# thomasgilgenast/hic3defdr

Hardware: AMD Instinct MI355X
Metric: pixels/sec through estimate_disp+lrt, 4 reps @10kb; max-|Δq| vs reference (higher is better)
Workload: dtype f64; 1 GPU; cfg2: per GPU 1 chrom x 20000 bins, 4 reps (2+2), dist_thresh_max 250, estimate_disp (qcml) + lrt on HBM-resident inputs; disp_pixels_rank0=3757837, disp_pixels_total=3757837, parallelism=dp1 (chromosome shards; in-kernel Brent searches)

## Files before the change

### hic3defdr_amd/csrc/h3d_api.hip

```cpp
#include <hip/hip_runtime.h>
#include <hipcub/hipcub.hpp>

#include <algorithm>
#include <chrono>
#include <cstdarg>
#include <cstdio>
#include <cstdlib>
#include <cstring>
#include <map>
#include <string>
#include <thread>
#include <type_traits>
#include <vector>

#include "h3d.h"
#include "h3d_ctx.h"
#include "h3d_errors.h"
#include "h3d_host.h"
#include "h3d_kernels.h"

using namespace h3d;
using namespace h3dint;
using h3derr::fail;

// ... 377 lines not shown
  int64_t n = 0;
  int R = 0, C = 0, D = 0;
  h3d_allreduce_fn reduce = nullptr;
  void* user = nullptr;
  const TableReq* treq = nullptr;
  int S = 0, mslot = 0;
  bool nll_full = false;
  std::vector<int> nrep;
  std::vector<int32_t> rep_idx;
  bool dev_tables = false;
  bool dual = false;
  HostStamps stamp;
  int32_t *raw_s = nullptr, *dist_s = nullptr;
  double *f_s = nullptr, *pd = nullptr;
  int64_t* d_seg = nullptr;
  std::vector<int64_t> seg_start;
  int n_chunks = 0;
  size_t max_items = 0;
  int64_t *d_cs = nullptr, *d_lpx = nullptr;
  int32_t *d_cl = nullptr, *d_cd = nullptr, *d_scb = nullptr, *d_sce = nullptr;
  int32_t *d_nrep = nullptr, *d_repidx = nullptr;
  SegState* d_st = nullptr;
  int32_t *d_list = nullptr, *d_meta = nullptr, *d_slb = nullptr, *d_sle = nullptr;
  double *d_partial = nullptr, *d_total = nullptr, *d_res = nullptr;
  int *d_flags = nullptr, *d_bad = nullptr, *d_queue = nullptr;
  GangTables gang;
  int32_t* h_meta = nullptr;
  double* h_resd = nullptr;
  SegState* h_sst = nullptr;
  int* h_bad = nullptr;
  bool have_res = false;
};

template <int M, bool NLL, bool kFull = false>
void launch_disp_work(const DispCall& c) {
  h3d_ctx* ctx = c.ctx;
  auto launch = [&](auto k) {
    hipLaunchKernelGGL(k, dim3(work_grid(ctx, k, c.max_items)), dim3(kBlock), 0, c.s, c.raw_s,
                       c.f_s, c.pd, c.n, c.d_cs, c.d_cl, c.d_cd, c.C, c.d_repidx, c.d_nrep,
                       c.d_st, c.d_flags, c.d_list, c.d_meta, c.d_partial, ctx->eq_static8);
  };
  {
    ProfScope ps(ctx, "disp_work", 0, 1);
    launch(k_disp_work<M, (M <= 8 ? 4 : 1), kEqualize, NLL, kFull>);
  }
  if constexpr (NLL) {
    ProfScope ps(ctx, "disp_nll", 0);
    launch(k_disp_work<M, 1, kNll>);
  }
}

template <typename K>
int radix_sort_pairs(h3d_ctx* ctx, const K* keys_in, K* keys_out, const int32_t* vals_in,
                     int32_t* vals_out, int64_t n, int begin_bit, int end_bit) {
  return cub_call(ctx, "cub_tmp", [&](void* tmp, size_t& bytes) {
    return hipcub::DeviceRadixSort::SortPairs(tmp, bytes, keys_in, keys_out, vals_in, vals_out,
                                              (int)n, begin_bit, end_bit, ctx->stream);
  });
}

int validate_and_plan(DispCall& c, const int32_t* cond_of_rep, int estimator) {
  h3d_ctx* ctx = c.ctx;
  const int64_t n = c.n;
  if (n < 0 || c.D < 1) return fail(H3D_EARG, "n=%lld D=%d", (long long)n, c.D);
  if (n > 0 && (!c.d_raw || !c.d_f || !c.d_dist)) return fail(H3D_EARG, "null device input");
  if (n >= (int64_t)1 << 31) return fail(H3D_EARG, "n=%lld exceeds 2^31 pixels per call", (long long)n);
  if (estimator != H3D_EST_QCML)
    return fail(H3D_EARG, "estimator %d: only qcml runs on the GPU path (the reference's cml/mme divide an int64 array in place and raise)", estimator);
  if (int rc = check_cond(cond_of_rep, c.R, c.C, &c.nrep, &c.rep_idx)) return rc;
  HIP_TRY(hipSetDevice(ctx->device));
  if (std::getenv("H3D_DEBUG")) {
    const hipError_t pe = hipGetLastError();
    if (pe != hipSuccess)
      fprintf(stderr, "[h3d] estimate_disp entry: pending HIP error %s\n", hipGetErrorString(pe));
  }
  c.s = ctx->stream;
  c.S = c.D * c.C;
// ... 290 lines not shown
int qcml_single_rank(DispCall& c) {
  h3d_ctx* ctx = c.ctx;
  if (c.n == 0) {
    Scratch sc{ctx};
    c.d_seg = sc.get<int64_t>("seg_start", c.D + 1);
    if (!sc.ok) return fail(H3D_ENOMEM, "brent scratch");
    HIP_TRY(hipMemsetAsync(c.d_seg, 0, (c.D + 1) * 8, c.s));
  }
  bool use_gang = ctx->brent_gang == 2 && c.n > 0;
  if (use_gang) {
    const int grc = with_width(c.mslot, false, [&](auto m, auto) {
      return gang_setup<decltype(m)::value>(ctx, c.seg_start, c.D, c.C, &c.gang);
    });
    if (grc == 1) use_gang = false;
    else if (grc) return grc;
  }
  int rounds = 0, batch = 5;
  while (true) {
    for (int b = 0; b < batch; ++b) {
      dbg_launch("before qcml iteration");
      with_width(c.mslot, c.nll_full, [&](auto m, auto full) {
        constexpr int M = decltype(m)::value;
        constexpr bool kFull = decltype(full)::value;
        auto brent = [&](const int32_t* gate_meta, int live_min, const int* gang_abort) {
          launch_brent<M, kFull>(ctx, c.pd, c.n, c.d_seg, c.S, c.C, c.d_repidx, c.d_nrep,
                                 c.d_st, c.d_flags, c.d_res, c.d_queue, gate_meta, live_min,
                                 gang_abort, true);
        };
        auto gang = [&](const int32_t* gate_meta, int live_max) {
          launch_brent_gang<M, kFull>(ctx, c.pd, c.n, c.d_seg, c.S, c.C, c.d_repidx, c.d_nrep,
                                      c.d_st, c.d_flags, c.d_res, c.d_queue + 1, c.gang,
                                      gate_meta, live_max, true);
        };
        launch_disp_work<M, false, kFull>(c);
        dbg_launch("equalize");
        if (c.dual) {
          brent(c.d_meta, ctx->n_cu, c.gang.abort);
          dbg_launch("k_brent (dual)");
          gang(c.d_meta, ctx->n_cu);
          dbg_launch("k_brent_gang (dual)");
        } else if (use_gang) {
          gang(nullptr, 0);
        } else {
          brent(nullptr, 0, nullptr);
        }
      });
      launch_seg_update(c, 0, 0);
      ++rounds;
    }
    const bool gangs = use_gang || c.dual;
    if (int rc = poll_single_rank(c, gangs)) return rc;
    if (std::getenv("H3D_DEBUG"))
      fprintf(stderr, "[h3d] qcml iterations=%d live_segments=%d gang=%d abort=%d\n", rounds,
              c.h_meta[3], use_gang ? 1 : c.dual ? 2 : 0, gangs ? c.h_meta[4] : 0);
    if (c.dual && c.h_meta[4]) {
      c.dual = false;
      ctx->gang_aborts += 1;
    }
    if (use_gang && c.h_meta[4]) {
      use_gang = false;
      ctx->gang_aborts += 1;
      continue;
    }
    if (c.h_meta[3] == 0) return 0;
    if (rounds > 2000) return fail(H3D_ENOCONV, "estimate_disp did not terminate");
    batch = 2;
  }
// ... 110 lines not shown
  }
  if (device < 0 || device >= n) {
    fail(H3D_EARG, "device %d of %d", device, n);
    return nullptr;
  }
  hipDeviceProp_t prop;
  if (hipGetDeviceProperties(&prop, device) != hipSuccess) {
    fail(H3D_EHIP, "hipGetDeviceProperties failed");
    return nullptr;
  }
  if (std::strncmp(prop.gcnArchName, "gfx950", 6) != 0) {
    fail(H3D_ENODEV, "device %d is %s, libh3d is built for gfx950", device,
         prop.gcnArchName);
    return nullptr;
  }
  if (hipSetDevice(device) != hipSuccess) {
    fail(H3D_EHIP, "hipSetDevice failed");
    return nullptr;
  }
  h3d_ctx* ctx = new h3d_ctx();
  ctx->device = device;
  ctx->n_cu = prop.multiProcessorCount;
  if (hipStreamCreateWithFlags(&ctx->own, hipStreamNonBlocking) != hipSuccess) {
    delete ctx;
    fail(H3D_EHIP, "stream create failed");
    return nullptr;
  }
  ctx->stream = ctx->own;
  if (const char* e = std::getenv("H3D_EQ_STATIC8"))
    ctx->eq_static8 = std::max(0, std::min(8, std::atoi(e)));
  if (const char* e = std::getenv("H3D_BRENT")) ctx->brent_gang = std::atoi(e);
  if (const char* e = std::getenv("H3D_BRENT_LDS_KB")) ctx->brent_lds_kb = std::atoi(e);
  if (const char* e = std::getenv("H3D_NLL_FULL")) ctx->nll_full = std::atoi(e);
  if (const char* e = std::getenv("H3D_GANG_P")) ctx->gang_px = std::atoi(e);
  if (hipMalloc((void**)&ctx->work_count, 2 * sizeof(unsigned long long)) != hipSuccess ||
      hipMemset(ctx->work_count, 0, 2 * sizeof(unsigned long long)) != hipSuccess) {
    (void)hipStreamDestroy(ctx->own);
    delete ctx;
    fail(H3D_ENOMEM, "counter allocation failed");
    return nullptr;
  }
  return ctx;
}

void h3d_close(h3d_ctx* ctx) {
  if (!ctx) return;
  (void)hipSetDevice(ctx->device);
  (void)hipStreamSynchronize(ctx->stream);
  prof_collect(ctx);
  for (auto& kv : ctx->bufs)
    if (kv.second.first) (void)hipFree(kv.second.first);
  for (auto e : ctx->event_pool) (void)hipEventDestroy(e);
  if (ctx->work_count) (void)hipFree(ctx->work_count);
  if (ctx->h_meta) (void)hipHostFree(ctx->h_meta);
  if (ctx->h_stage_done) (void)hipEventDestroy(ctx->h_stage_done);
  if (ctx->bounce_ev) (void)hipEventDestroy(ctx->bounce_ev);
  if (ctx->own) (void)hipStreamDestroy(ctx->own);
  delete ctx;
}

int h3d_set_stream(h3d_ctx* ctx, void* stream) {
  if (!ctx) return fail(H3D_EARG, "null ctx");
  ctx->stream = stream ? (hipStream_t)stream : ctx->own;
  return 0;
}

// ... 228 lines not shown
```

### hic3defdr_amd/csrc/h3d_ctx.h

```cpp
#pragma once

#include <hip/hip_runtime.h>

#include <cstdint>
#include <map>
#include <string>
#include <vector>

#include "h3d.h"
#include "h3d_errors.h"

#define HIP_TRY(expr)                                                      \
  do {                                                                     \
    hipError_t e_ = (expr);                                                \
    if (e_ != hipSuccess)                                                  \
      return h3derr::fail(H3D_EHIP, "%s failed: %s (%s:%d)", #expr,        \
                          hipGetErrorString(e_), __FILE__, __LINE__);      \
  } while (0)

namespace h3d {

struct PrepUnion {
  int R = 0, n_bins = 0;
  int64_t n_entries = 0, n_px = 0;
// ... 47 lines not shown
  }
};

}

struct h3d_ctx {
  int device = 0;
  hipStream_t own = nullptr;
  hipStream_t stream = nullptr;
  int n_cu = 256;
  std::map<const void*, int> resident;
  int prof = 0;
  std::map<std::string, h3dint::ProfEntry> stats;
  std::vector<std::pair<std::string, std::pair<hipEvent_t, hipEvent_t>>> pending;
  std::vector<int64_t> pending_units;
  std::vector<hipEvent_t> event_pool;
  std::map<std::string, std::pair<void*, size_t>> bufs;
  h3d::PrepUnion prep;
  unsigned long long* work_count = nullptr;
  int32_t* h_meta = nullptr;
  h3dint::PinnedBuf h_stage;
  h3dint::PinnedBuf h_res;
  hipEvent_t h_stage_done = nullptr;
  h3dint::PinnedBuf bounce;
  size_t bounce_off = 0;
  hipEvent_t bounce_ev = nullptr;
  hipStream_t bounce_stream = nullptr;
  h3dint::PinnedBuf land;
  int eq_static8 = 4;
  int brent_gang = 1;
  int gang_aborts = 0;
  int brent_lds_kb = 128;
  int nll_full = 1;
  double qcml_tol = 1e-4;
  int gang_px = 0;
  int gang_epoch = 0;
  void* gang_tag_buf = nullptr;
  size_t gang_tag_cap = 0;
  int last_S = 0;
  h3dint::TablePending tab_pending;
};

namespace h3dint {

constexpr int kLaunchBlock = 256;
constexpr int kTableMaxD = 1024;

void* scratch(h3d_ctx* ctx, const char* slot, size_t bytes);
void* scratch_keep(h3d_ctx* ctx, const char* slot, size_t bytes, size_t keep);

struct Scratch {
  h3d_ctx* ctx;
  bool ok = true;
  template <typename T>
  T* get(const char* slot, size_t count) {
    T* p = (T*)scratch(ctx, slot, count * sizeof(T));
    ok = ok && p;
    return p;
  }
  template <typename T>
  T* keep(const char* slot, size_t count, size_t keep_count) {
    T* p = (T*)scratch_keep(ctx, slot, count * sizeof(T), keep_count * sizeof(T));
    ok = ok && p;
    return p;
  }
};
// ... 60 lines not shown
```

### hic3defdr_amd/csrc/h3d_hosttest.cpp

```cpp
#include <cstdint>
#include <vector>

#include "h3d_model.h"
#include "h3d_special.h"

namespace {
constexpr int M = h3d::kMaxReps;
}

extern "C" {

#define H3DT_UNARY(name, fn)                                   \
  void h3dt_##name(int64_t n, const double* x, double* out) { \
    for (int64_t i = 0; i < n; ++i) out[i] = h3d::fn(x[i]);   \
  }
#define H3DT_BINARY(name, fn)                                     \
  void h3dt_##name(int64_t n, const double* a, const double* x,  \
                   double* out) {                                 \
    for (int64_t i = 0; i < n; ++i) out[i] = h3d::fn(a[i], x[i]); \
  }

H3DT_UNARY(lgam, lgam)
H3DT_UNARY(lgam_nll, lgam_nll)
H3DT_UNARY(log_fast, log_fast)
H3DT_UNARY(ndtr, ndtr)
H3DT_UNARY(ndtri, ndtri)
H3DT_UNARY(log1pmx, log1pmx)
H3DT_UNARY(lgam1p, lgam1p)
H3DT_BINARY(igam, igam)
H3DT_BINARY(igamc, igamc)
H3DT_BINARY(igami, igami)
H3DT_BINARY(igamci, igamci)
H3DT_BINARY(chi2_sf, chi2_sf)

int h3dt_fit_mu(int64_t n, int r, const int32_t* x, const double* b,
                const double* alpha, double* mu) {
  int bad = 0;
  for (int64_t i = 0; i < n; ++i) {
    double xs[M], bs[M], as[M];
    for (int k = 0; k < r; ++k) {
      xs[k] = x[i * r + k];
      bs[k] = b[i * r + k];
      as[k] = alpha[i * r + k];
    }
    int st = 0;
    mu[i] = h3d::fit_mu<M>(xs, bs, as, r, ~0u, &st);
    bad |= st;
  }
  return bad;
}

void h3dt_q2q(int64_t n, const double* x, const double* mu_in,
              const double* mu_out, const double* alpha, double* out) {
  for (int64_t i = 0; i < n; ++i) {
    double mi = mu_in[i], mo = mu_out[i];
    out[i] = h3d::q2q(x[i], &mi, &mo, alpha[i]);
  }
}

int h3dt_equalize(int64_t n, int r, const int32_t* x, const double* f,
                  double alpha, double* out) {
  int bad = 0;
  for (int64_t i = 0; i < n; ++i) {
    double xs[M], fs[M], ps[M];
    for (int k = 0; k < r; ++k) {
      xs[k] = x[i * r + k];
      fs[k] = f[i * r + k];
    }
    bad |= h3d::equalize_pixel<M>(xs, fs, r, alpha, ps);
    for (int k = 0; k < r; ++k) out[i * r + k] = ps[k];
  }
  return bad;
}

int h3dt_nll_terms(int64_t n, int r, const double* pseudo, double delta, int mode,
                   double* out) {
  if (r < 1 || r > M || mode < 0 || mode > 2) return -1;
  const h3d::NllConst kc = h3d::nll_const(delta, r);
  for (int64_t i = 0; i < n; ++i) {
    double ps[M];
    for (int k = 0; k < M; ++k) ps[k] = k < r ? pseudo[i * r + k] : 0.0;
    out[i] = mode == 2   ? h3d::nll_pixel_large<M>(ps, r, kc)
             : mode == 1 ? h3d::nll_pixel_mid<M>(ps, r, kc)
                         : h3d::nll_pixel<M>(ps, r, kc);
  }
  return 0;
}

int h3dt_lrt(int64_t n, int R, int C, const int32_t* raw, const double* f,
             const double* disp_wide, const int32_t* cond_of_rep, int refit,
// ... 100 lines not shown
```

### hic3defdr_amd/csrc/h3d_kernels.h

```cpp
#pragma once

#include <hip/hip_runtime.h>

#include <cstdint>

#include "h3d_model.h"

namespace h3d {

constexpr int kChunk = 256;
constexpr int kBlock = 256;
constexpr int kWavesPerBlock = kBlock / 64;
template <int M>
constexpr int brent_block() {
  return M >= 16 ? 512 : 1024;
}

__device__ inline double wave_sum(double v) {
#pragma unroll
  for (int off = 32; off > 0; off >>= 1) v += __shfl_xor(v, off, 64);
  return v;
}

__device__ inline double block_sum(double v, double* lds) {
#pragma unroll
  for (int off = 32; off > 0; off >>= 1) v += __shfl_xor(v, off, 64);
  const int lane = threadIdx.x & 63, wid = threadIdx.x >> 6;
  if (lane == 0) lds[wid] = v;
  __syncthreads();
  double t = 0.0;
  if (threadIdx.x == 0) {
    const int nw = (blockDim.x + 63) >> 6;
    for (int w = 0; w < nw; ++w) t += lds[w];
  }
  return t;
}

// ... 220 lines not shown
        for (int j = 0; j < G; ++j) {
          task_seg[t0 + c * G + j] = d * C + c;
          task_g[t0 + c * G + j] = j;
        }
    }
    if (d < D) {
      scb[d] = b0;
      sce[d] = b0 + nch;
      const int64_t a = seg[d];
      for (int j = 0; j < nch; ++j) {
        cs[b0 + j] = a + (int64_t)j * kChunk;
        cl[b0 + j] = (int32_t)min((int64_t)kChunk, len - (int64_t)j * kChunk);
        cd[b0 + j] = d;
      }
      for (int c = 0; c < C; ++c) {
        seg_init(&st[d * C + c], (long long)len, n_rep[c], tol);
        lpx[d * C + c] = len;
      }
    }
    __syncthreads();
    if (threadIdx.x == 0) {
      s_carry += tot;
      s_tcarry += ttot;
    }
    __syncthreads();
  }
  if (task_seg)
    for (int t = s_tcarry + threadIdx.x; t < task_len; t += 1024) task_seg[t] = -1;
}

constexpr int kTaskHeadStride = 32;
constexpr int kWorkMetaInts = kTaskHeadStride * 17;

template <int M, int W, int PH, bool NLL = true, bool kFull = false>
__global__ __launch_bounds__(kBlock, W) void k_disp_work(
    const int32_t* __restrict__ raw_s, const double* __restrict__ f_s,
    double* __restrict__ pd, int64_t n, const int64_t* __restrict__ chunk_start,
    const int32_t* __restrict__ chunk_len, const int32_t* __restrict__ chunk_d,
    int C, const int32_t* __restrict__ rep_idx ,
    const int32_t* __restrict__ n_rep , const SegState* __restrict__ st,
    int* __restrict__ seg_flags, const int32_t* __restrict__ list,
    int32_t* __restrict__ meta ,
    double* __restrict__ partial, int static8) {
  const int beg = (PH == kEqualize) ? 0 : meta[2];
  const int end = (PH == kEqualize) ? meta[2] : meta[0];
  constexpr int kWv = kBlock / 64;
  const int lane = threadIdx.x & 63;
  const int64_t t0 = (int64_t)beg * kWv, t1 = (int64_t)end * kWv;
  const int64_t wt = (int64_t)gridDim.x * kWv;
  const int64_t tdyn = (t1 - t0 < 2 * wt) ? t1 : t0 + ((t1 - t0) / wt) * static8 / 8 * wt;
  const int64_t tl = t1 - tdyn;
  int32_t* heads = meta + kTaskHeadStride * (1 + (PH == kEqualize ? 0 : 8));
  const int grp = blockIdx.x & 7;
  unsigned spent = 0u;
  auto take = [&]() -> int64_t {
    if (tl <= 0) return t1;
#pragma unroll 1
    for (int k = 0; k < 8; ++k) {
      const int p = (grp + k) & 7;
      if ((spent >> p) & 1u) continue;
      const int64_t pb = tdyn + tl * p / 8, pe = tdyn + tl * (p + 1) / 8;
      int got = 0;
      if (lane == 0) got = atomicAdd(heads + kTaskHeadStride * p, 1);
      got = __shfl(got, 0, 64);
      if (pb + got < pe) return pb + got;
      spent |= 1u << p;
    }
    return t1;
  };
  __shared__ LogTab s_tab[kLogTabLen];
  for (int k = threadIdx.x; k < kLogTabLen; k += kBlock) s_tab[k] = kLogTab[k];
  __syncthreads();
  int64_t t = t0 + (int64_t)blockIdx.x * kWv + (threadIdx.x >> 6);
  if (t >= tdyn) t = take();
  for (; t < t1; t = (t + wt < tdyn) ? t + wt : take()) {
    const int w = (int)(t / kWv);
    const int q = (int)(t - (int64_t)w * kWv);
    const int item = list[w];
    const int chunk = item / C, c = item - chunk * C;
    const int s = chunk_d[chunk] * C + c;
    constexpr int phase = PH;
    const int nr = kFull ? M : n_rep[c];
    double term = 0.0;
    const int i = q * 64 + lane;
    H3D_SEC_BEGIN(t_task);
    if (i < chunk_len[chunk] && nr < 8) {
      constexpr int MS = M < 8 ? M : 8;
      const int64_t px = chunk_start[chunk] + i;
      const NllConst kc = st[s].k;
      const int32_t* ri = rep_idx + c * kMaxReps;
      double lgsum = 0.0, z = 0.0;
      if (phase == kEqualize) {
        const double alpha = st[s].disp;
        double x[MS], f[MS], as[MS], lf[MS];
#pragma unroll
        for (int k = 0; k < MS; ++k) {
          const bool on = k < nr;
          x[k] = on ? (double)raw_s[(int64_t)ri[k] * n + px] : 0.0;
          f[k] = on ? f_s[(int64_t)ri[k] * n + px] : 1.0;
          lf[k] = on ? log_fast_checked(f[k], s_tab) : 0.0;
          as[k] = alpha;
        }
        int fl = 0;
        H3D_SEC_BEGIN(t_fit);
        const double f_mean = exp_fast(np_sum<MS>(lf, nr) / nr) - 0.0;
        const double mu = fit_mu<MS>(x, f, as, nr, ~0u, &fl, s_tab);
        H3D_SEC_END(0, t_fit);
        if (fl) atomicOr(&seg_flags[s], fl);
        const double mu_out0 = mu * f_mean;
        int fc = nr;
        unsigned up = 0u, lo = 0u;
#pragma unroll
        for (int k = MS - 1; k >= 0; --k)
          if (k < nr) {
            const double mi = mu * f[k];
            if (!(mi >= 0.25 && mu_out0 >= 0.25)) fc = k;
            if (x[k] >= mi)
              up |= 1u << k;
            else
              lo |= 1u << k;
          }
        LgamCache cache;
#pragma unroll 1
        for (int j = 0; j < nr; ++j) {
          int k;
          if (up) {
            k = __builtin_ctz(up);
            up &= up - 1u;
          } else {
            k = __builtin_ctz(lo);
            lo &= lo - 1u;
          }
          const int64_t o = (int64_t)ri[k] * n + px;
          double mu_in = mu * f_s[o];
          double mu_out = (k > fc) ? 0.25 : mu_out0;
          H3D_SEC_BEGIN(t_q2q);
          pd[o] = q2q((double)raw_s[o], &mu_in, &mu_out, alpha, &cache, s_tab);
          H3D_SEC_END(13, t_q2q);
        }
      }
      if (phase == kEqualize) H3D_SEC_END(14, t_task);
      if constexpr (!NLL) continue;
      {
        double d[MS];
#pragma unroll
        for (int k = 0; k < MS; ++k)
          d[k] = (k < nr) ? pd[(int64_t)ri[k] * n + px] : 0.0;
#pragma unroll 1
        for (int k = 0; k < nr; ++k) {
          const double dk = d[0];
#pragma unroll
          for (int j = 0; j + 1 < MS; ++j) d[j] = d[j + 1];
          lgsum += lgam_nll(dk + kc.r, s_tab);
          z += dk;
        }
      }
      term = lgsum + kc.lg_nr - lgam_nll(z + kc.nr, s_tab) - kc.n_lg_r;
    } else if (M >= 8 && i < chunk_len[chunk]) {
      const int64_t px = chunk_start[chunk] + i;
      double d[M];
      int ri[M];
#pragma unroll
      for (int k = 0; k < M; ++k) ri[k] = (k < nr) ? rep_idx[c * kMaxReps + k] : 0;
      if (phase == kEqualize) {
        double x[M], f[M];
#pragma unroll
        for (int k = 0; k < M; ++k) {
          if (k < nr) {
            x[k] = (double)raw_s[(int64_t)ri[k] * n + px];
            f[k] = f_s[(int64_t)ri[k] * n + px];
// ... 750 lines not shown
```

### hic3defdr_amd/csrc/h3d_model.h

```cpp
#pragma once

#include <cmath>

#include "h3d_special.h"

namespace h3d {

constexpr int kMaxReps = 32;
constexpr int kMaxConds = 8;

constexpr int kFlagNoRoot = 1;
constexpr int kFlagNoConv = 2;
constexpr int kFlagBrentFail = 4;
constexpr int kFlagQcmlGuard = 8;
constexpr int kFlagBadInput = 16;

template <int M>
H3D_HD double np_sum(const double* v, int n) {
  if (n < 8) {
    double res = 0.0;
#pragma unroll
    for (int i = 0; i < (M < 8 ? M : 8); ++i)
      if (i < n) res += v[i];
    return res;
// ... 150 lines not shown
H3D_HD double gamma_cdf(double x, double shape, double scale) {
  const double xs = x / scale;
  if (xs <= 0.0) return 0.0;
  return igam(shape, xs);
}
H3D_HD double gamma_isf(double q, double shape, double scale) {
  if (q != q) return NAN;
  if (q == 0.0) return INFINITY;
  if (q == 1.0) return 0.0;
  return igamci(shape, q) * scale;
}
H3D_HD double gamma_ppf(double q, double shape, double scale) {
  if (q != q) return NAN;
  if (q == 0.0) return 0.0;
  if (q == 1.0) return INFINITY;
  return igami(shape, q) * scale;
}

struct LgamCache {
  double a = -1.0, lga = 0.0;
};

H3D_HD double lgam_q2q(double a, const LogTab* tab = kLogTab) { return lgam_nll(a, tab); }

H3D_HD double lgam_cached(double a, LgamCache* c, const LogTab* tab = kLogTab) {
  if (!c) return lgam_q2q(a, tab);
  if (a != c->a) {
    c->a = a;
    c->lga = lgam_q2q(a, tab);
  }
  return c->lga;
}

H3D_HD double q2q_core(double x, double mi, double mo, double alpha,
                       double lga_out, LgamCache* cache, const LogTab* tab = kLogTab);

H3D_HD double q2q(double x, double* mu_in, double* mu_out, double alpha,
                  LgamCache* cache = nullptr, const LogTab* tab = kLogTab) {
  if (!((*mu_in >= 0.25) && (*mu_out >= 0.25))) {
    *mu_in = 0.25;
    *mu_out = 0.25;
  }
  return q2q_core(x, *mu_in, *mu_out, alpha, NAN, cache, tab);
}

H3D_HD double q2q_core(double x, double mi, double mo, double alpha,
                       double lga_out, LgamCache* cache, const LogTab* tab) {
  H3D_SEC_BEGIN(t_setup);
  const double r_in = 1 + alpha * mi, r_out = 1 + alpha * mo;
  const double v_in = mi * r_in, v_out = mo * r_out;
  const double rr_in = recip_fast(r_in);
  const double a_in = mi * rr_in, a_out = div_fast(mo, r_out);
  const bool right = x >= mi;
  const double dxm = x - mi;
  const double rv_in = recip_fast(v_in);
  const double zh2 = dxm * dxm * rv_in * 0.5;
  const bool under = zh2 > kMaxLog;
  double qn;
  if (dxm != dxm || rv_in != rv_in)
    qn = NAN;
  else if (right && dxm > 0.0 && under)
    qn = INFINITY;
  else if (!right && dxm < 0.0 && under)
    qn = -INFINITY;
  else
    qn = dxm * sqrt(v_out * rv_in) + mo;
  const double xs = x * rr_in;
  H3D_SEC_END(1, t_setup);
  double tg;
  if (xs <= 0.0) {
    tg = right ? 1.0 : 0.0;
  } else {
    double P, Q, fac;
    H3D_SEC_BEGIN(t_lg);
    const double lga_in = lgam_q2q(a_in, tab);
    H3D_SEC_END(2, t_lg);
    igam_pq(a_in, xs, lga_in, &P, &Q, &fac, right ? 1 : 0, tab, 3);
    tg = right ? Q : P;
  }
  double qg;
  if (tg != tg) {
    qg = NAN;
  } else if (tg == 0.0) {
    qg = right ? INFINITY : 0.0;
  } else if (tg == 1.0) {
    qg = right ? 0.0 : INFINITY;
  } else {
    double guess = -1.0;
    H3D_SEC_BEGIN(t_wh);
    if (a_in >= 1.0 && a_out >= 1.0) {
      const double m_in = 1.0 - recip_fast(9.0 * a_in);
      const double m_out = 1.0 - recip_fast(9.0 * a_out);
#if defined(__HIP_DEVICE_COMPILE__)
      const float zz = (cbrtf((float)div_fast(xs, a_in)) - (float)m_in) *
                       sqrtf((float)(9.0 * a_in));
      const double y = m_out + (double)(zz * rsqrtf((float)(9.0 * a_out)));
#else
      const double zz = (cbrt(div_fast(xs, a_in)) - m_in) * sqrt(9.0 * a_in);
      const double y = m_out + div_fast(zz, sqrt(9.0 * a_out));
#endif
      if (y > 0.0) guess = a_out * y * y * y;
    }
    H3D_SEC_END(5, t_wh);
    H3D_SEC_BEGIN(t_lgo);
    const double lga = (lga_out == lga_out) ? lga_out : lgam_cached(a_out, cache, tab);
    H3D_SEC_END(6, t_lgo);
    H3D_SEC_BEGIN(t_inv);
    qg = igam_inv(a_out, tg, right, lga, guess, tab) * r_out;
    H3D_SEC_END(7, t_inv);
  }
  double pc = (qn + qg) / 2;
  if (!(pc >= 0.0)) pc = 0.0;
  return pc;
}

template <int M>
H3D_HD_INLINE int equalize_pixel(const double* x, const double* f, int n, double alpha,
                          double* out, const LogTab* tab = kLogTab) {
  double lf[M], as[M];
#pragma unroll
  for (int k = 0; k < M; ++k) {
    lf[k] = (k < n) ? log_fast_checked(f[k], tab) : 0.0;
    as[k] = alpha;
  }
  const double f_mean = exp_fast(np_sum<M>(lf, n) / n) - 0.0;
  int st = 0;
  const double mu = fit_mu<M>(x, f, as, n, ~0u, &st, tab);
  double mu_out = mu * f_mean;
  LgamCache cache;
#pragma unroll
  for (int k = 0; k < M; ++k)
    if (k < n) {
      double mu_in = mu * f[k];
      out[k] = q2q(x[k], &mu_in, &mu_out, alpha, &cache, tab);
    }
  return st;
}

H3D_HD double logpmf(double k, double m, double phi) {
  const double r = 1.0 / phi;
  return lgam(r + k) - lgam(k + 1) - lgam(r) + r * log(r) - r * log(r + m) +
         k * log(m) - k * log(r + m);
}

template <int M, int CM, typename TX>
H3D_HD int lrt_pixel(const TX* x, const double* f, const double* a,
                     const int* cond, int R, int C, bool refit, double* p,
                     double* llr, double* mu0, double* mu1,
                     const LogTab* tab = kLogTab) {
  int st = 0;
#pragma unroll 1
  for (int t = 0; t <= C; ++t) {
    unsigned mask = 0u;
#pragma unroll
    for (int k = 0; k < M; ++k)
      if (k < R && (t == 0 || cond[k] == t - 1)) mask |= (1u << k);
    double mu;
    if (refit) {
      mu = fit_mu<M>(x, f, a, R, mask, &st);
    } else {
      int cnt = 0;
#pragma unroll
      for (int k = 0; k < M; ++k) cnt += (k < R && ((mask >> k) & 1u)) ? 1 : 0;
      NpSumStream q(cnt);
      int j = 0;
#pragma unroll
      for (int k = 0; k < M; ++k)
// ... 266 lines not shown
```

### hic3defdr_amd/csrc/h3d_selftest.hip

```cpp
#include <hip/hip_runtime.h>

#include <algorithm>
#include <cmath>
#include <cstdint>
#include <cstdio>
#include <vector>

#include "h3d_model.h"
#include "h3d_special.h"

namespace {

constexpr int M = h3d::kMaxReps;
constexpr int kBlock = 256;

enum Op {
  kLgam, kLgamNll, kLogFast, kNdtr, kNdtri, kLog1pmx, kLgam1p,
  kIgam, kIgamc, kIgami, kIgamci, kChi2Sf
};

template <int OP>
__device__ double unary_op(double x) {
  if constexpr (OP == kLgam) return h3d::lgam(x);
  else if constexpr (OP == kLgamNll) return h3d::lgam_nll(x);
// ... 30 lines not shown
}

__global__ void k_fit_mu(int64_t n, int r, const int32_t* __restrict__ x,
                         const double* __restrict__ b,
                         const double* __restrict__ alpha, double* __restrict__ mu,
                         int* __restrict__ status) {
  int st_all = 0;
  for (int64_t i = blockIdx.x * (int64_t)blockDim.x + threadIdx.x; i < n;
       i += (int64_t)gridDim.x * blockDim.x) {
    double xs[M], bs[M], as[M];
#pragma unroll
    for (int k = 0; k < M; ++k) {
      const bool on = k < r;
      xs[k] = on ? (double)x[i * r + k] : 0.0;
      bs[k] = on ? b[i * r + k] : 1.0;
      as[k] = on ? alpha[i * r + k] : 1.0;
    }
    int st = 0;
    mu[i] = h3d::fit_mu<M>(xs, bs, as, r, ~0u, &st);
    st_all |= st;
  }
  if (st_all) atomicOr(status, st_all);
}

__global__ void k_q2q(int64_t n, const double* __restrict__ x,
                      const double* __restrict__ mu_in,
                      const double* __restrict__ mu_out,
                      const double* __restrict__ alpha, double* __restrict__ out) {
  for (int64_t i = blockIdx.x * (int64_t)blockDim.x + threadIdx.x; i < n;
       i += (int64_t)gridDim.x * blockDim.x) {
    double mi = mu_in[i], mo = mu_out[i];
    out[i] = h3d::q2q(x[i], &mi, &mo, alpha[i]);
  }
}

__global__ void k_equalize_nll(int64_t n, int r, const int32_t* __restrict__ x,
                               const double* __restrict__ f, double alpha,
                               int do_equalize, double* __restrict__ pseudo,
                               h3d::NllConst kc, double* __restrict__ term,
                               int* __restrict__ status) {
  int st_all = 0;
  for (int64_t i = blockIdx.x * (int64_t)blockDim.x + threadIdx.x; i < n;
       i += (int64_t)gridDim.x * blockDim.x) {
    double ps[M];
    if (do_equalize) {
      double xs[M], fs[M];
#pragma unroll
      for (int k = 0; k < M; ++k) {
        const bool on = k < r;
        xs[k] = on ? (double)x[i * r + k] : 0.0;
        fs[k] = on ? f[i * r + k] : 1.0;
      }
      st_all |= h3d::equalize_pixel<M>(xs, fs, r, alpha, ps);
#pragma unroll
      for (int k = 0; k < M; ++k)
        if (k < r) pseudo[i * r + k] = ps[k];
    } else {
#pragma unroll
      for (int k = 0; k < M; ++k) ps[k] = (k < r) ? pseudo[i * r + k] : 0.0;
    }
    if (term) term[i] = h3d::nll_pixel<M>(ps, r, kc);
  }
  if (st_all) atomicOr(status, st_all);
}

__global__ void k_nll_terms(int64_t n, int r, const double* __restrict__ pseudo,
// ... 126 lines not shown
H3DT_UNARY(ndtr, kNdtr)
H3DT_UNARY(ndtri, kNdtri)
H3DT_UNARY(log1pmx, kLog1pmx)
H3DT_UNARY(lgam1p, kLgam1p)
H3DT_BINARY(igam, kIgam)
H3DT_BINARY(igamc, kIgamc)
H3DT_BINARY(igami, kIgami)
H3DT_BINARY(igamci, kIgamci)
H3DT_BINARY(chi2_sf, kChi2Sf)

int h3dt_fit_mu(int64_t n, int r, const int32_t* x, const double* b,
                const double* alpha, double* mu) {
  if (r < 1 || r > M) return -1;
  Dev<int32_t> dx(x, n * r);
  Dev<double> db(b, n * r), da(alpha, n * r), dmu(nullptr, n);
  Dev<int> dst(nullptr, 1);
  hipLaunchKernelGGL(k_fit_mu, dim3(grid_of(n)), dim3(kBlock), 0, 0, n, r, dx.p, db.p,
                     da.p, dmu.p, dst.p);
  int st = 0;
  if (!sync_ok()) return -2;
  dmu.to_host(mu);
  dst.to_host(&st);
  return g_failed ? -2 : st;
}

void h3dt_q2q(int64_t n, const double* x, const double* mu_in,
              const double* mu_out, const double* alpha, double* out) {
  Dev<double> dx(x, n), di(mu_in, n), dout_(mu_out, n), dal(alpha, n), d(nullptr, n);
  hipLaunchKernelGGL(k_q2q, dim3(grid_of(n)), dim3(kBlock), 0, 0, n, dx.p, di.p, dout_.p,
                     dal.p, d.p);
  if (sync_ok()) d.to_host(out);
  if (g_failed)
    for (int64_t i = 0; i < n; ++i) out[i] = NAN;
}

int h3dt_equalize(int64_t n, int r, const int32_t* x, const double* f,
                  double alpha, double* out) {
  if (r < 1 || r > M) return -1;
  Dev<int32_t> dx(x, n * r);
  Dev<double> df(f, n * r), dp(nullptr, n * r);
  Dev<int> dst(nullptr, 1);
  hipLaunchKernelGGL(k_equalize_nll, dim3(grid_of(n)), dim3(kBlock), 0, 0, n, r, dx.p,
                     df.p, alpha, 1, dp.p, h3d::NllConst{}, (double*)nullptr, dst.p);
  int st = 0;
  if (!sync_ok()) return -2;
  dp.to_host(out);
  dst.to_host(&st);
  return g_failed ? -2 : st;
}

int h3dt_nll_terms(int64_t n, int r, const double* pseudo, double delta, int mode,
                   double* out) {
  if (r < 1 || r > M || mode < 0 || mode > 2) return -1;
  Dev<double> dp(pseudo, n * r), dout_(nullptr, n);
  const h3d::NllConst kc = h3d::nll_const(delta, r);
  hipLaunchKernelGGL(k_nll_terms, dim3(grid_of(n)), dim3(kBlock), 0, 0, n, r, dp.p, kc, mode,
                     dout_.p);
  if (!sync_ok()) return -2;
  dout_.to_host(out);
  return g_failed ? -2 : 0;
}

int h3dt_lrt(int64_t n, int R, int C, const int32_t* raw, const double* f,
             const double* disp_wide, const int32_t* cond_of_rep, int refit,
             double* p, double* llr, double* mu0, double* mu1) {
  if (R < 1 || R > M || C < 1 || C > h3d::kMaxConds) return -1;
// ... 50 lines not shown
```

### hic3defdr_amd/csrc/h3d_special.h

```cpp
#pragma once

#include <cmath>
#include <cstdint>

#if defined(__clang__)
#pragma clang fp contract(off)
#endif

#if defined(__HIPCC__)
#define H3D_HD __host__ __device__ inline
#define H3D_HD_COLD __host__ __device__ inline __attribute__((noinline))
#define H3D_HD_INLINE __host__ __device__ inline __attribute__((always_inline))
#else
#define H3D_HD inline
#define H3D_HD_COLD inline
#define H3D_HD_INLINE inline
#endif

#if defined(H3D_INSTRUMENT) && !defined(__HIP_DEVICE_COMPILE__)
namespace h3d {
struct Stats {
  long pq, cf, su, ser, cf_it, su_it, ser_it, fac_l1, l1_it, inv, halley, wh,
      lgam, lgam_small, lgam_it, fit, fit_it;
};
// ... 716 lines not shown
constexpr int kTaylorK = 12;

H3D_HD bool igam_taylor_ok(double a, double xe, double h) {
  const double rx = recip_fast(xe);
  const double u = h * rx;
  return xe > 0.0 && fabs(u) <= 0.05 &&
         fabs(((a - 1.0) * rx - 1.0) * h) <= 0.4 &&
         fabs(a - 1.0) * u * u <= 0.25;
}

H3D_HD void igam_step_taylor(double a, double xe, double h, double* dint,
                             double* ratio) {
#if defined(__clang__)
#pragma clang fp contract(fast)
#endif
  constexpr int K = kTaylorK;
  const double b = a - 1.0;
  const double u = h * recip_fast(xe);
  const double c0 = b - xe;
  double em1 = 0.0, e = 1.0;
  double in = 1.0, ex = 1.0;
#pragma unroll
  for (int k = 0; k < K; ++k) {
    const double en = u * ((c0 - k) * e - h * em1) * (1.0 / (k + 1));
    em1 = e;
    e = en;
    in += e * (1.0 / (k + 2));
    ex += e;
  }
  *dint = in * h;
  *ratio = ex;
}

H3D_HD double igam_inv(double a, double t, bool upper, double lga,
                       double guess = -1.0, const LogTab* tab = kLogTab) {
  H3D_STAT(inv, 1);
  H3D_STAT(wh, guess > 0.0);
  if (t > 0.9) {
    t = 1.0 - t;
    upper = !upper;
  }
  H3D_SEC_BEGIN(t_dm);
  double x = (guess > 0.0) ? guess
                           : upper ? find_inverse_gamma(a, 1.0 - t, t, lga)
                                   : find_inverse_gamma(a, t, 1.0 - t, lga);
  H3D_SEC_END(10, t_dm);
  double xe = -1.0, Fe = 0.0, dPe = 0.0;
  for (int i = 0; i < 8; ++i) {
    H3D_STAT(halley, 1);
    double F, dP;
    const double h = x - xe;
    H3D_SEC_BEGIN(t_tay);
    const bool tay = igam_taylor_ok(a, xe, h);
    if (tay) {
      double dint, ratio;
      igam_step_taylor(a, xe, h, &dint, &ratio);
      const double dPint = dPe * dint;
      F = upper ? Fe - dPint : Fe + dPint;
      dP = dPe * ratio;
    }
    H3D_SEC_END(11, t_tay);
    if (!tay) {
      double P, Q, fac;
      igam_pq(a, x, lga, &P, &Q, &fac, upper ? 1 : 0, tab, 8);
      if (fac == 0.0) return x;
      F = (upper ? Q : P) - t;
      dP = fac / x;
      xe = x;
      Fe = F;
      dPe = dP;
    }
    H3D_SEC_BEGIN(t_hal);
    const bool nrm = fabs(dP) >= 0x1p-1000 && x >= 0x1p-1000;
    double f_fp, fpp_fp;
    if (nrm) {
      f_fp = div_fast(upper ? -F : F, dP);
      fpp_fp = -1.0 + div_fast(a - 1, x);
    } else {
      f_fp = upper ? -F / dP : F / dP;
      fpp_fp = -1.0 + (a - 1) / x;
    }
    double xn = is_inf(fpp_fp) ? x - f_fp
                               : x - div_fast(f_fp, 1.0 - 0.5 * f_fp * fpp_fp);
    if (!(xn > 0.0)) xn = 0.5 * x;
    const double dx = fabs(xn - x);
    x = xn;
    H3D_SEC_END(12, t_hal);
    if (dx <= 1e-6 * x) break;
  }
  return x;
}

H3D_HD double igami(double a, double p) {
  if (a != a || p != p) return NAN;
  if (a < 0.0 || p < 0.0 || p > 1.0) return NAN;
  if (p == 0.0) return 0.0;
  if (p == 1.0) return INFINITY;
  return igam_inv(a, p, false, lgam(a));
}

H3D_HD double igamci(double a, double q) {
  if (a != a || q != q) return NAN;
  if (a < 0.0 || q < 0.0 || q > 1.0) return NAN;
  if (q == 0.0) return INFINITY;
  if (q == 1.0) return 0.0;
  return igam_inv(a, q, true, lgam(a));
}

H3D_HD double chi2_sf(double df, double x);

H3D_HD_COLD double chi2_sf_cold(double df, double x) { return chi2_sf(df, x); }

H3D_HD double chi2_sf(double df, double x) {
  if (x != x) return NAN;
  if (x <= 0.0) return 1.0;
  if (df == 1.0) return erfc(sqrt(x / 2.0));
  if (df == 2.0) return exp(-x / 2.0);
  return igamc(df / 2.0, x / 2.0);
}
// ... 3 lines not shown
```

Baseline: 705.2 million pixels/s.

## Share one igam_pq call site between forward CDF and first inverse evaluation

Restructures the q2q gamma path so the forward incomplete-gamma evaluation and the first Halley evaluation of the inverse run through a single igam_pq call in a two-trip loop. Later re-evaluations move to a noinline cold helper. The aim is to cut divergent code and instruction-cache footprint in the equalize kernel. It also switches the work-distribution indices to 32-bit and makes the wave index wave-uniform via readfirstlane, guarded by a size check. The rework adds loop control overhead and may change register allocation; the new path is enabled by default but can be turned off with an environment variable.

```diff
diff --git a/hic3defdr_amd/csrc/h3d_api.hip b/hic3defdr_amd/csrc/h3d_api.hip
--- a/hic3defdr_amd/csrc/h3d_api.hip
+++ b/hic3defdr_amd/csrc/h3d_api.hip
@@ -433,7 +433,7 @@
   bool have_res = false;
 };
 
-template <int M, bool NLL, bool kFull = false>
+template <int M, bool NLL, bool kFull = false, bool kEval1 = false>
 void launch_disp_work(const DispCall& c) {
   h3d_ctx* ctx = c.ctx;
   auto launch = [&](auto k) {
@@ -443,7 +443,7 @@
   };
   {
     ProfScope ps(ctx, "disp_work", 0, 1);
-    launch(k_disp_work<M, (M <= 8 ? 4 : 1), kEqualize, NLL, kFull>);
+    launch(k_disp_work<M, (M <= 8 ? 4 : 1), kEqualize, NLL, kFull, kEval1>);
   }
   if constexpr (NLL) {
     ProfScope ps(ctx, "disp_nll", 0);
@@ -800,7 +800,10 @@
                                       c.d_st, c.d_flags, c.d_res, c.d_queue + 1, c.gang,
                                       gate_meta, live_max, true);
         };
-        launch_disp_work<M, false, kFull>(c);
+        if (ctx->eq_eval1 && c.max_items < ((size_t)1 << 31) / (8 * kWavesPerBlock))
+          launch_disp_work<M, false, kFull, true>(c);
+        else
+          launch_disp_work<M, false, kFull>(c);
         dbg_launch("equalize");
         if (c.dual) {
           brent(c.d_meta, ctx->n_cu, c.gang.abort);
@@ -977,6 +980,7 @@
   if (const char* e = std::getenv("H3D_BRENT")) ctx->brent_gang = std::atoi(e);
   if (const char* e = std::getenv("H3D_BRENT_LDS_KB")) ctx->brent_lds_kb = std::atoi(e);
   if (const char* e = std::getenv("H3D_NLL_FULL")) ctx->nll_full = std::atoi(e);
+  if (const char* e = std::getenv("H3D_EQ_EVAL1")) ctx->eq_eval1 = std::atoi(e);
   if (const char* e = std::getenv("H3D_GANG_P")) ctx->gang_px = std::atoi(e);
   if (hipMalloc((void**)&ctx->work_count, 2 * sizeof(unsigned long long)) != hipSuccess ||
       hipMemset(ctx->work_count, 0, 2 * sizeof(unsigned long long)) != hipSuccess) {
diff --git a/hic3defdr_amd/csrc/h3d_ctx.h b/hic3defdr_amd/csrc/h3d_ctx.h
--- a/hic3defdr_amd/csrc/h3d_ctx.h
+++ b/hic3defdr_amd/csrc/h3d_ctx.h
@@ -103,6 +103,7 @@
   int gang_aborts = 0;
   int brent_lds_kb = 128;
   int nll_full = 1;
+  int eq_eval1 = 1;
   double qcml_tol = 1e-4;
   int gang_px = 0;
   int gang_epoch = 0;
diff --git a/hic3defdr_amd/csrc/h3d_hosttest.cpp b/hic3defdr_amd/csrc/h3d_hosttest.cpp
--- a/hic3defdr_amd/csrc/h3d_hosttest.cpp
+++ b/hic3defdr_amd/csrc/h3d_hosttest.cpp
@@ -1,4 +1,6 @@
+#define H3D_INSTRUMENT 1
 #include <cstdint>
+#include <cstring>
 #include <vector>
 
 #include "h3d_model.h"
@@ -56,6 +58,43 @@
     double mi = mu_in[i], mo = mu_out[i];
     out[i] = h3d::q2q(x[i], &mi, &mo, alpha[i]);
   }
+}
+
+int h3dt_q2q_form(int64_t n, const double* x, const double* mu_in,
+                  const double* mu_out, const double* alpha, int form, double* out,
+                  int64_t* paths) {
+  if (form != 0 && form != 1) return -1;
+  for (int64_t i = 0; i < n; ++i) {
+    double mi = mu_in[i], mo = mu_out[i];
+    h3d::Stats s;
+    memset(&s, 0, sizeof s);
+    h3d::g_stats = &s;
+    out[i] = form ? h3d::q2q<true>(x[i], &mi, &mo, alpha[i])
+                  : h3d::q2q<false>(x[i], &mi, &mo, alpha[i]);
+    h3d::g_stats = nullptr;
+    if (paths) {
+      const long v[6] = {s.ser, s.su, s.cf, s.inv, s.wh, s.halley};
+      for (int j = 0; j < 6; ++j) paths[i * 6 + j] = v[j];
+    }
+  }
+  return 0;
+}
+
+int h3dt_equalize_form(int64_t n, int r, const int32_t* x, const double* f,
+                       double alpha, int form, double* out) {
+  if (r < 1 || r > 8 || (form != 0 && form != 1)) return -1;
+  int bad = 0;
+  for (int64_t i = 0; i < n; ++i) {
+    double xs[8], fs[8], ps[8];
+    for (int k = 0; k < 8; ++k) {
+      xs[k] = k < r ? (double)x[i * r + k] : 0.0;
+      fs[k] = k < r ? f[i * r + k] : 1.0;
+    }
+    bad |= form ? h3d::equalize_pixel<8, true>(xs, fs, r, alpha, ps)
+                : h3d::equalize_pixel<8, false>(xs, fs, r, alpha, ps);
+    for (int k = 0; k < r; ++k) out[i * r + k] = ps[k];
+  }
+  return bad;
 }
 
 int h3dt_equalize(int64_t n, int r, const int32_t* x, const double* f,
diff --git a/hic3defdr_amd/csrc/h3d_kernels.h b/hic3defdr_amd/csrc/h3d_kernels.h
--- a/hic3defdr_amd/csrc/h3d_kernels.h
+++ b/hic3defdr_amd/csrc/h3d_kernels.h
@@ -3,6 +3,7 @@
 #include <hip/hip_runtime.h>
 
 #include <cstdint>
+#include <type_traits>
 
 #include "h3d_model.h"
 
@@ -289,7 +290,7 @@
 constexpr int kTaskHeadStride = 32;
 constexpr int kWorkMetaInts = kTaskHeadStride * 17;
 
-template <int M, int W, int PH, bool NLL = true, bool kFull = false>
+template <int M, int W, int PH, bool NLL = true, bool kFull = false, bool kEval1 = false>
 __global__ __launch_bounds__(kBlock, W) void k_disp_work(
     const int32_t* __restrict__ raw_s, const double* __restrict__ f_s,
     double* __restrict__ pd, int64_t n, const int64_t* __restrict__ chunk_start,
@@ -303,20 +304,21 @@
   const int end = (PH == kEqualize) ? meta[2] : meta[0];
   constexpr int kWv = kBlock / 64;
   const int lane = threadIdx.x & 63;
-  const int64_t t0 = (int64_t)beg * kWv, t1 = (int64_t)end * kWv;
-  const int64_t wt = (int64_t)gridDim.x * kWv;
-  const int64_t tdyn = (t1 - t0 < 2 * wt) ? t1 : t0 + ((t1 - t0) / wt) * static8 / 8 * wt;
-  const int64_t tl = t1 - tdyn;
+  using TI = std::conditional_t<kEval1, int32_t, int64_t>;
+  const TI t0 = (TI)beg * kWv, t1 = (TI)end * kWv;
+  const TI wt = (TI)gridDim.x * kWv;
+  const TI tdyn = (t1 - t0 < 2 * wt) ? t1 : t0 + ((t1 - t0) / wt) * static8 / 8 * wt;
+  const TI tl = t1 - tdyn;
   int32_t* heads = meta + kTaskHeadStride * (1 + (PH == kEqualize ? 0 : 8));
   const int grp = blockIdx.x & 7;
   unsigned spent = 0u;
-  auto take = [&]() -> int64_t {
+  auto take = [&]() -> TI {
     if (tl <= 0) return t1;
 #pragma unroll 1
     for (int k = 0; k < 8; ++k) {
       const int p = (grp + k) & 7;
       if ((spent >> p) & 1u) continue;
-      const int64_t pb = tdyn + tl * p / 8, pe = tdyn + tl * (p + 1) / 8;
+      const TI pb = tdyn + tl * p / 8, pe = tdyn + tl * (p + 1) / 8;
       int got = 0;
       if (lane == 0) got = atomicAdd(heads + kTaskHeadStride * p, 1);
       got = __shfl(got, 0, 64);
@@ -328,11 +330,12 @@
   __shared__ LogTab s_tab[kLogTabLen];
   for (int k = threadIdx.x; k < kLogTabLen; k += kBlock) s_tab[k] = kLogTab[k];
   __syncthreads();
-  int64_t t = t0 + (int64_t)blockIdx.x * kWv + (threadIdx.x >> 6);
+  TI t = t0 + (TI)blockIdx.x * kWv + (TI)(threadIdx.x >> 6);
   if (t >= tdyn) t = take();
   for (; t < t1; t = (t + wt < tdyn) ? t + wt : take()) {
-    const int w = (int)(t / kWv);
-    const int q = (int)(t - (int64_t)w * kWv);
+    int w = (int)(t / kWv);
+    if constexpr (kEval1) w = __builtin_amdgcn_readfirstlane(w);
+    const int q = (int)(t - (TI)w * kWv);
     const int item = list[w];
     const int chunk = item / C, c = item - chunk * C;
     const int s = chunk_d[chunk] * C + c;
@@ -392,7 +395,7 @@
           double mu_in = mu * f_s[o];
           double mu_out = (k > fc) ? 0.25 : mu_out0;
           H3D_SEC_BEGIN(t_q2q);
-          pd[o] = q2q((double)raw_s[o], &mu_in, &mu_out, alpha, &cache, s_tab);
+          pd[o] = q2q<kEval1>((double)raw_s[o], &mu_in, &mu_out, alpha, &cache, s_tab);
           H3D_SEC_END(13, t_q2q);
         }
       }
diff --git a/hic3defdr_amd/csrc/h3d_model.h b/hic3defdr_amd/csrc/h3d_model.h
--- a/hic3defdr_amd/csrc/h3d_model.h
+++ b/hic3defdr_amd/csrc/h3d_model.h
@@ -206,18 +206,118 @@
   return c->lga;
 }
 
+template <bool kEval1 = false>
 H3D_HD double q2q_core(double x, double mi, double mo, double alpha,
                        double lga_out, LgamCache* cache, const LogTab* tab = kLogTab);
 
+template <bool kEval1 = false>
 H3D_HD double q2q(double x, double* mu_in, double* mu_out, double alpha,
                   LgamCache* cache = nullptr, const LogTab* tab = kLogTab) {
   if (!((*mu_in >= 0.25) && (*mu_out >= 0.25))) {
     *mu_in = 0.25;
     *mu_out = 0.25;
   }
-  return q2q_core(x, *mu_in, *mu_out, alpha, NAN, cache, tab);
-}
-
+  return q2q_core<kEval1>(x, *mu_in, *mu_out, alpha, NAN, cache, tab);
+}
+
+H3D_HD double q2q_wh_guess(double xs, double a_in, double a_out) {
+  double guess = -1.0;
+  if (a_in >= 1.0 && a_out >= 1.0) {
+    const double m_in = 1.0 - recip_fast(9.0 * a_in);
+    const double m_out = 1.0 - recip_fast(9.0 * a_out);
+#if defined(__HIP_DEVICE_COMPILE__)
+    const float zz = (cbrtf((float)div_fast(xs, a_in)) - (float)m_in) *
+                     sqrtf((float)(9.0 * a_in));
+    const double y = m_out + (double)(zz * rsqrtf((float)(9.0 * a_out)));
+#else
+    const double zz = (cbrt(div_fast(xs, a_in)) - m_in) * sqrt(9.0 * a_in);
+    const double y = m_out + div_fast(zz, sqrt(9.0 * a_out));
+#endif
+    if (y > 0.0) guess = a_out * y * y * y;
+  }
+  return guess;
+}
+
+H3D_HD double q2q_gamma(double xs, bool right, double a_in, double a_out, double r_out,
+                        double lga_out, LgamCache* cache, const LogTab* tab) {
+  double tg;
+  if (xs <= 0.0) {
+    tg = right ? 1.0 : 0.0;
+  } else {
+    double P, Q, fac;
+    H3D_SEC_BEGIN(t_lg);
+    const double lga_in = lgam_q2q(a_in, tab);
+    H3D_SEC_END(2, t_lg);
+    igam_pq(a_in, xs, lga_in, &P, &Q, &fac, right ? 1 : 0, tab, 3);
+    tg = right ? Q : P;
+  }
+  double qg;
+  if (tg != tg) {
+    qg = NAN;
+  } else if (tg == 0.0) {
+    qg = right ? INFINITY : 0.0;
+  } else if (tg == 1.0) {
+    qg = right ? 0.0 : INFINITY;
+  } else {
+    H3D_SEC_BEGIN(t_wh);
+    const double guess = q2q_wh_guess(xs, a_in, a_out);
+    H3D_SEC_END(5, t_wh);
+    H3D_SEC_BEGIN(t_lgo);
+    const double lga = (lga_out == lga_out) ? lga_out : lgam_cached(a_out, cache, tab);
+    H3D_SEC_END(6, t_lgo);
+    H3D_SEC_BEGIN(t_inv);
+    qg = igam_inv(a_out, tg, right, lga, guess, tab) * r_out;
+    H3D_SEC_END(7, t_inv);
+  }
+  return qg;
+}
+
+H3D_HD double q2q_gamma_e1(double xs, bool right, double a_in, double a_out, double r_out,
+                           double lga_out, LgamCache* cache, const LogTab* tab) {
+  double ea = a_in, ex = xs, elga = 0.0;
+  bool etail = right, live = !(xs <= 0.0);
+  if (live) {
+    H3D_SEC_BEGIN(t_lg);
+    elga = lgam_q2q(ea, tab);
+    H3D_SEC_END(2, t_lg);
+  }
+  double ev = etail ? 1.0 : 0.0, efac = 0.0, t = 0.0;
+#pragma unroll 1
+  for (int trip = 0;; ++trip) {
+    if (live) {
+      double P, Q;
+      igam_pq(ea, ex, elga, &P, &Q, &efac, etail ? 1 : 0, tab, trip ? 8 : 3);
+      ev = etail ? Q : P;
+    }
+    if (trip) break;
+    live = ev == ev && ev != 0.0 && ev != 1.0;
+    if (live) {
+      H3D_SEC_BEGIN(t_wh);
+      const double guess = q2q_wh_guess(ex, ea, a_out);
+      H3D_SEC_END(5, t_wh);
+      H3D_SEC_BEGIN(t_lgo);
+      elga = (lga_out == lga_out) ? lga_out : lgam_cached(a_out, cache, tab);
+      H3D_SEC_END(6, t_lgo);
+      t = ev;
+      ex = igam_inv_start(a_out, &t, &etail, elga, guess);
+      ea = a_out;
+    }
+  }
+  H3D_SEC_BEGIN(t_inv);
+  double qg;
+  if (live)
+    qg = igam_inv_rest(ea, t, etail, elga, ex, ev, efac) * r_out;
+  else if (ev != ev)
+    qg = NAN;
+  else if (ev == 0.0)
+    qg = etail ? INFINITY : 0.0;
+  else
+    qg = etail ? 0.0 : INFINITY;
+  H3D_SEC_END(7, t_inv);
+  return qg;
+}
+
+template <bool kEval1>
 H3D_HD double q2q_core(double x, double mi, double mo, double alpha,
                        double lga_out, LgamCache* cache, const LogTab* tab) {
   H3D_SEC_BEGIN(t_setup);
@@ -241,54 +341,17 @@
     qn = dxm * sqrt(v_out * rv_in) + mo;
   const double xs = x * rr_in;
   H3D_SEC_END(1, t_setup);
-  double tg;
-  if (xs <= 0.0) {
-    tg = right ? 1.0 : 0.0;
-  } else {
-    double P, Q, fac;
-    H3D_SEC_BEGIN(t_lg);
-    const double lga_in = lgam_q2q(a_in, tab);
-    H3D_SEC_END(2, t_lg);
-    igam_pq(a_in, xs, lga_in, &P, &Q, &fac, right ? 1 : 0, tab, 3);
-    tg = right ? Q : P;
-  }
   double qg;
-  if (tg != tg) {
-    qg = NAN;
-  } else if (tg == 0.0) {
-    qg = right ? INFINITY : 0.0;
-  } else if (tg == 1.0) {
-    qg = right ? 0.0 : INFINITY;
-  } else {
-    double guess = -1.0;
-    H3D_SEC_BEGIN(t_wh);
-    if (a_in >= 1.0 && a_out >= 1.0) {
-      const double m_in = 1.0 - recip_fast(9.0 * a_in);
-      const double m_out = 1.0 - recip_fast(9.0 * a_out);
-#if defined(__HIP_DEVICE_COMPILE__)
-      const float zz = (cbrtf((float)div_fast(xs, a_in)) - (float)m_in) *
-                       sqrtf((float)(9.0 * a_in));
-      const double y = m_out + (double)(zz * rsqrtf((float)(9.0 * a_out)));
-#else
-      const double zz = (cbrt(div_fast(xs, a_in)) - m_in) * sqrt(9.0 * a_in);
-      const double y = m_out + div_fast(zz, sqrt(9.0 * a_out));
-#endif
-      if (y > 0.0) guess = a_out * y * y * y;
-    }
-    H3D_SEC_END(5, t_wh);
-    H3D_SEC_BEGIN(t_lgo);
-    const double lga = (lga_out == lga_out) ? lga_out : lgam_cached(a_out, cache, tab);
-    H3D_SEC_END(6, t_lgo);
-    H3D_SEC_BEGIN(t_inv);
-    qg = igam_inv(a_out, tg, right, lga, guess, tab) * r_out;
-    H3D_SEC_END(7, t_inv);
-  }
+  if constexpr (kEval1)
+    qg = q2q_gamma_e1(xs, right, a_in, a_out, r_out, lga_out, cache, tab);
+  else
+    qg = q2q_gamma(xs, right, a_in, a_out, r_out, lga_out, cache, tab);
   double pc = (qn + qg) / 2;
   if (!(pc >= 0.0)) pc = 0.0;
   return pc;
 }
 
-template <int M>
+template <int M, bool kEval1 = false>
 H3D_HD_INLINE int equalize_pixel(const double* x, const double* f, int n, double alpha,
                           double* out, const LogTab* tab = kLogTab) {
   double lf[M], as[M];
@@ -306,7 +369,7 @@
   for (int k = 0; k < M; ++k)
     if (k < n) {
       double mu_in = mu * f[k];
-      out[k] = q2q(x[k], &mu_in, &mu_out, alpha, &cache, tab);
+      out[k] = q2q<kEval1>(x[k], &mu_in, &mu_out, alpha, &cache, tab);
     }
   return st;
 }
diff --git a/hic3defdr_amd/csrc/h3d_selftest.hip b/hic3defdr_amd/csrc/h3d_selftest.hip
--- a/hic3defdr_amd/csrc/h3d_selftest.hip
+++ b/hic3defdr_amd/csrc/h3d_selftest.hip
@@ -86,6 +86,40 @@
     double mi = mu_in[i], mo = mu_out[i];
     out[i] = h3d::q2q(x[i], &mi, &mo, alpha[i]);
   }
+}
+
+template <bool kEval1>
+__global__ void k_q2q_form(int64_t n, const double* __restrict__ x,
+                           const double* __restrict__ mu_in,
+                           const double* __restrict__ mu_out,
+                           const double* __restrict__ alpha, double* __restrict__ out) {
+  for (int64_t i = blockIdx.x * (int64_t)blockDim.x + threadIdx.x; i < n;
+       i += (int64_t)gridDim.x * blockDim.x) {
+    double mi = mu_in[i], mo = mu_out[i];
+    out[i] = h3d::q2q<kEval1>(x[i], &mi, &mo, alpha[i]);
+  }
+}
+
+template <bool kEval1>
+__global__ void k_equalize_form(int64_t n, int r, const int32_t* __restrict__ x,
+                                const double* __restrict__ f, double alpha,
+                                double* __restrict__ pseudo, int* __restrict__ status) {
+  int st_all = 0;
+  for (int64_t i = blockIdx.x * (int64_t)blockDim.x + threadIdx.x; i < n;
+       i += (int64_t)gridDim.x * blockDim.x) {
+    double xs[8], fs[8], ps[8];
+#pragma unroll
+    for (int k = 0; k < 8; ++k) {
+      const bool on = k < r;
+      xs[k] = on ? (double)x[i * r + k] : 0.0;
+      fs[k] = on ? f[i * r + k] : 1.0;
+    }
+    st_all |= h3d::equalize_pixel<8, kEval1>(xs, fs, r, alpha, ps);
+#pragma unroll
+    for (int k = 0; k < 8; ++k)
+      if (k < r) pseudo[i * r + k] = ps[k];
+  }
+  if (st_all) atomicOr(status, st_all);
 }
 
 __global__ void k_equalize_nll(int64_t n, int r, const int32_t* __restrict__ x,
@@ -278,6 +312,42 @@
   if (sync_ok()) d.to_host(out);
   if (g_failed)
     for (int64_t i = 0; i < n; ++i) out[i] = NAN;
+}
+
+int h3dt_q2q_form(int64_t n, const double* x, const double* mu_in,
+                  const double* mu_out, const double* alpha, int form, double* out,
+                  int64_t* paths) {
+  (void)paths;
+  if (form != 0 && form != 1) return -1;
+  Dev<double> dx(x, n), di(mu_in, n), dout_(mu_out, n), dal(alpha, n), d(nullptr, n);
+  if (form)
+    hipLaunchKernelGGL(k_q2q_form<true>, dim3(grid_of(n)), dim3(kBlock), 0, 0, n, dx.p, di.p,
+                       dout_.p, dal.p, d.p);
+  else
+    hipLaunchKernelGGL(k_q2q_form<false>, dim3(grid_of(n)), dim3(kBlock), 0, 0, n, dx.p, di.p,
+                       dout_.p, dal.p, d.p);
+  if (!sync_ok()) return -2;
+  d.to_host(out);
+  return g_failed ? -2 : 0;
+}
+
+int h3dt_equalize_form(int64_t n, int r, const int32_t* x, const double* f,
+                       double alpha, int form, double* out) {
+  if (r < 1 || r > 8 || (form != 0 && form != 1)) return -1;
+  Dev<int32_t> dx(x, n * r);
+  Dev<double> df(f, n * r), dp(nullptr, n * r);
+  Dev<int> dst(nullptr, 1);
+  if (form)
+    hipLaunchKernelGGL(k_equalize_form<true>, dim3(grid_of(n)), dim3(kBlock), 0, 0, n, r, dx.p,
+                       df.p, alpha, dp.p, dst.p);
+  else
+    hipLaunchKernelGGL(k_equalize_form<false>, dim3(grid_of(n)), dim3(kBlock), 0, 0, n, r,
+                       dx.p, df.p, alpha, dp.p, dst.p);
+  int st = 0;
+  if (!sync_ok()) return -2;
+  dp.to_host(out);
+  dst.to_host(&st);
+  return g_failed ? -2 : st;
 }
 
 int h3dt_equalize(int64_t n, int r, const int32_t* x, const double* f,
diff --git a/hic3defdr_amd/csrc/h3d_special.h b/hic3defdr_amd/csrc/h3d_special.h
--- a/hic3defdr_amd/csrc/h3d_special.h
+++ b/hic3defdr_amd/csrc/h3d_special.h
@@ -772,6 +772,24 @@
   *ratio = ex;
 }
 
+H3D_HD double igam_inv_halley(double a, bool upper, double x, double F, double dP,
+                              double* dx) {
+  const bool nrm = fabs(dP) >= 0x1p-1000 && x >= 0x1p-1000;
+  double f_fp, fpp_fp;
+  if (nrm) {
+    f_fp = div_fast(upper ? -F : F, dP);
+    fpp_fp = -1.0 + div_fast(a - 1, x);
+  } else {
+    f_fp = upper ? -F / dP : F / dP;
+    fpp_fp = -1.0 + (a - 1) / x;
+  }
+  double xn = is_inf(fpp_fp) ? x - f_fp
+                             : x - div_fast(f_fp, 1.0 - 0.5 * f_fp * fpp_fp);
+  if (!(xn > 0.0)) xn = 0.5 * x;
+  *dx = fabs(xn - x);
+  return xn;
+}
+
 H3D_HD double igam_inv(double a, double t, bool upper, double lga,
                        double guess = -1.0, const LogTab* tab = kLogTab) {
   H3D_STAT(inv, 1);
@@ -811,20 +829,77 @@
       dPe = dP;
     }
     H3D_SEC_BEGIN(t_hal);
-    const bool nrm = fabs(dP) >= 0x1p-1000 && x >= 0x1p-1000;
-    double f_fp, fpp_fp;
-    if (nrm) {
-      f_fp = div_fast(upper ? -F : F, dP);
-      fpp_fp = -1.0 + div_fast(a - 1, x);
-    } else {
-      f_fp = upper ? -F / dP : F / dP;
-      fpp_fp = -1.0 + (a - 1) / x;
-    }
-    double xn = is_inf(fpp_fp) ? x - f_fp
-                               : x - div_fast(f_fp, 1.0 - 0.5 * f_fp * fpp_fp);
-    if (!(xn > 0.0)) xn = 0.5 * x;
-    const double dx = fabs(xn - x);
-    x = xn;
+    double dx;
+    x = igam_inv_halley(a, upper, x, F, dP, &dx);
+    H3D_SEC_END(12, t_hal);
+    if (dx <= 1e-6 * x) break;
+  }
+  return x;
+}
+
+
+H3D_HD double igam_inv_start(double a, double* t, bool* upper, double lga, double guess) {
+  H3D_STAT(inv, 1);
+  H3D_STAT(wh, guess > 0.0);
+  if (*t > 0.9) {
+    *t = 1.0 - *t;
+    *upper = !*upper;
+  }
+  H3D_SEC_BEGIN(t_dm);
+  const double x = (guess > 0.0) ? guess
+                   : *upper      ? find_inverse_gamma(a, 1.0 - *t, *t, lga)
+                                 : find_inverse_gamma(a, *t, 1.0 - *t, lga);
+  H3D_SEC_END(10, t_dm);
+  return x;
+}
+
+struct IgamTail {
+  double v, fac;
+};
+H3D_HD_COLD IgamTail igam_tail_cold(double a, double x, double lga, bool upper) {
+  double P, Q;
+  IgamTail r;
+  igam_pq(a, x, lga, &P, &Q, &r.fac, upper ? 1 : 0, kLogTab, 8);
+  r.v = upper ? Q : P;
+  return r;
+}
+
+H3D_HD double igam_inv_rest(double a, double t, bool upper, double lga, double x,
+                            double v, double fac) {
+  H3D_STAT(halley, 1);
+  if (fac == 0.0) return x;
+  double F = v - t, dP = fac / x;
+  double xe = x, Fe = F, dPe = dP;
+  double dx;
+  H3D_SEC_BEGIN(t_hal0);
+  x = igam_inv_halley(a, upper, x, F, dP, &dx);
+  H3D_SEC_END(12, t_hal0);
+  if (dx <= 1e-6 * x) return x;
+#pragma unroll 1
+  for (int i = 1; i < 8; ++i) {
+    H3D_STAT(halley, 1);
+    const double h = x - xe;
+    H3D_SEC_BEGIN(t_tay);
+    const bool tay = igam_taylor_ok(a, xe, h);
+    if (tay) {
+      double dint, ratio;
+      igam_step_taylor(a, xe, h, &dint, &ratio);
+      const double dPint = dPe * dint;
+      F = upper ? Fe - dPint : Fe + dPint;
+      dP = dPe * ratio;
+    }
+    H3D_SEC_END(11, t_tay);
+    if (!tay) {
+      const IgamTail e = igam_tail_cold(a, x, lga, upper);
+      if (e.fac == 0.0) return x;
+      F = e.v - t;
+      dP = e.fac / x;
+      xe = x;
+      Fe = F;
+      dPe = dP;
+    }
+    H3D_SEC_BEGIN(t_hal);
+    x = igam_inv_halley(a, upper, x, F, dP, &dx);
     H3D_SEC_END(12, t_hal);
     if (dx <= 1e-6 * x) break;
   }
```

Result: no change. 711.9 million pixels/s, median of 6 (+1.0%).
